# evalf/nutils

Measured on AMD Instinct MI355X. Metric: elements assembled/sec (global stiffness K), higher is better.
Workload: dtype f64; 1 GPU; 3D Poisson stiffness, 128^3 structured hex, p=1, 2x2x2 Gauss, iso geometry (BASELINE.json configs[1]); nelems_per_gpu=2097152, nnz_per_gpu=57066625, kernel=k_p1hex_skew<16,16,false,false>, parallelism=single GPU, launch=hipGraph replay (20 steps per graph), settle_steps=600

## Files before the change

### nutils_amd/csrc/nh_assemble_p1hex.hip

```cpp
#include "nh_common.h"
#include <algorithm>
#include <type_traits>
#include <cstdio>
#include <cstdlib>

namespace {

#ifdef NH_ABLATION
#define DEBUG(p) ((p).debug)
#else
#define DEBUG(p) 0
#endif

struct P1Args {
  int n0, n1, n2;
  int lay0, lay1;
  int pl0, pl1;
  const double *verts;
  double origin[3], scale[3];
  double n[2][2];
  double c[3][2];
  double wk[2][2][2];
  double wm[2][2][2];
  int hasm;
  const double *qmass;
  double *values;
  const double *qscale;
  const double *u;
  double *out;
  int accumulate;
  int nbj, nbk;
  long long *tdbg;
  int wbnd;
  int debug;
};

__device__ __forceinline__ int len_of(int X, int N) { return (X > 0) + 1 + (X < N - 1); }
__device__ __forceinline__ i64 cum_of(int X, int N) { return X == 0 ? 0 : 3 * (i64)X - 1; }

__device__ __forceinline__ double fast_rcp(double d) {
  double r = __builtin_amdgcn_rcp(d);
  r = fma(fma(-d, r, 1.), r, r);
  r = fma(fma(-d, r, 1.), r, r);
  return r;
}

__device__ __forceinline__ void lds_barrier() { asm volatile("s_waitcnt lgkmcnt(0)\n\ts_barrier" ::: "memory"); }

struct ElemTables {
  double R0[3][3], R1[3][3], R2[3][3];
  double W01[2][2][3], W02[2][2][3], W12[2][2][3];
  double Mm[3][3][3];
};

__device__ __forceinline__ double element_entry(const ElemTables &T, int a, int bb) {
  const int a0 = a >> 2, a1 = (a >> 1) & 1, a2 = a & 1;
  const int b0 = bb >> 2, b1 = (bb >> 1) & 1, b2 = bb & 1;
  const int p0 = a0 + b0, p1 = a1 + b1, p2 = a2 + b2;
  const double s00 = (a0 == b0) ? 1. : -1., s11 = (a1 == b1) ? 1. : -1., s22 = (a2 == b2) ? 1. : -1.;
  const double s01 = (a0 == b1) ? 1. : -1., s10 = (b0 == a1) ? 1. : -1.;
  const double s02 = (a0 == b2) ? 1. : -1., s20 = (b0 == a2) ? 1. : -1.;
  const double s12 = (a1 == b2) ? 1. : -1., s21 = (b1 == a2) ? 1. : -1.;
  return s00 * T.R0[p1][p2] + s11 * T.R1[p0][p2] + s22 * T.R2[p0][p1] + s01 * T.W01[b0][a1][p2] + s10 * T.W01[a0][b1][p2] +
         s02 * T.W02[b0][a2][p1] + s20 * T.W02[a0][b2][p1] + s12 * T.W12[b1][a2][p0] + s21 * T.W12[a1][b2][p0] + T.Mm[p0][p1][p2];
}

template <int TJ, int TK, int L, int VPT, int VW>
__device__ __forceinline__ void load_vertex_tile(const P1Args &p, bool valid, int J0, int K0, int L0, int tid, double (&V)[VPT][VW]) {
  constexpr int NT = L * TJ * TK, VJ = TJ + 1, VK = TK + 1, NV = (L + 1) * VJ * VK;
  const int N0 = p.n0 + 1, N1 = p.n1 + 1, N2 = p.n2 + 1;
#pragma unroll
  for (int k = 0; k < VPT; ++k) {
    const int v = tid + k * NT;
    const int c = v % VK, bb = (v / VK) % VJ, a = v / (VK * VJ);
    const int I = L0 + a, J = J0 - 1 + bb, K = K0 - 1 + c;
#pragma unroll
    for (int w = 0; w < VW; ++w) V[k][w] = 0.;
    if (valid && v < NV && I >= 0 && I < N0 && J >= 0 && J < N1 && K >= 0 && K < N2) {
      const i64 node = ((i64)I * N1 + J) * N2 + K;
      const double *src = p.verts + node * 3;
      V[k][0] = src[0];
      V[k][1] = src[1];
      V[k][2] = src[2];
      if constexpr (VW == 4) V[k][3] = p.u[node];
    }
  }
}

template <int TJ, int TK, int L, bool VEC, bool MASS, bool COEF>
__global__ __launch_bounds__(L * TJ * TK) void k_p1hex_march(P1Args p) {
#ifdef NH_ABLATION
  long long tacc[12] = {0, 0, 0, 0, 0, 0, 0, 0, 0, 0, 0, 0}, tprev = clock64();
#define NH_TICK(i) { const long long tnow = clock64(); tacc[i] += tnow - tprev; tprev = tnow; }
#else
#define NH_TICK(i)
#endif
  constexpr int NT = L * TJ * TK, NP = L + 2, OJ = TJ - 1, OK = TK - 1;
  constexpr int NS = VEC ? 1 : 15;
  constexpr int VW = VEC ? 4 : 3;
  constexpr int VJ = TJ + 1, VK = TK + 1, RP = VJ * VK, PS = (RP * NS + 1) & ~1, NV = (L + 1) * VJ * VK, VPT = (NV + NT - 1) / NT;
  extern __shared__ __attribute__((aligned(16))) double lds[];
  double *acc = lds;
  double *vbuf = lds + NP * PS;
  const int tid = threadIdx.x;
  const int N0 = p.n0 + 1, N1 = p.n1 + 1, N2 = p.n2 + 1;
  const int NPL = p.pl1 - p.pl0;
  const i64 U = (i64)p.nbj * p.nbk * NPL;
  const unsigned wg = gridDim.x % 8 == 0 ? (blockIdx.x % 8) * (gridDim.x / 8) + blockIdx.x / 8 : blockIdx.x;
  i64 u = U * wg / gridDim.x;
  const i64 u1 = U * (wg + 1) / gridDim.x;
  if (u >= u1) return;
  auto slot_of = [](int P) { return (int)((unsigned)(P + 2 * NP) % NP) * PS; };
  int col = (int)(u / NPL), A = p.pl0 + (int)(u % NPL), B = (int)min((i64)p.pl1, A + (u1 - u)), L0 = A - 1;
  double V[VPT][VW];
  load_vertex_tile<TJ, TK, L, VPT, VW>(p, true, (col / p.nbk) * OJ, (col % p.nbk) * OK, L0, tid, V);
  for (int t = tid; t < NP * PS / 2; t += NT) reinterpret_cast<double2 *>(acc)[t] = make_double2(0., 0.);
  auto stage_vertex_tile = [&]() {
#pragma unroll
    for (int k = 0; k < VPT; ++k) {
// ... 148 lines not shown
          const int nl = half ? 7 : 8;
          if (l < 202) {
#pragma unroll
            for (int pl = 0; pl < 2; ++pl) {
              char *lp = base + pl * (8 * (3 * T1 * T2)) + 16 * l;
#pragma unroll
              for (int i = 0; i < 8; ++i)
                if (i < nl) {
                  const double2 v = make_double2(a0[pl][i], a1[pl][i]);
                  __builtin_memcpy(lp + i * (2 * stride8), &v, 16);
                }
            }
          } else if (l == 202) {
#pragma unroll
            for (int pl = 0; pl < 2; ++pl) {
              char *lp = base + pl * (8 * (3 * T1 * T2)) + 16 * l;
#pragma unroll
              for (int i = 0; i < 8; ++i)
                if (i < nl) *reinterpret_cast<double *>(lp + i * (2 * stride8)) = a0[pl][i];
            }
          }
        } else if (L == 2 && !lowJ && !highJ && Pe - Pb == 2 && Pb > 0 && Pe < N0) {
          const int flag = 1 | 2 | loK << 2 | 8 | 16 | hiK << 5;
          const unsigned voff8 = 8u * (unsigned)(9 * cumK + ((dI + 1) * 3 + (dJ + 1)) * lenK + (dK + loK));
          const i64 stride8 = 8 * (i64)(9 * (int)T2);
          if (kact && (flag & need) == need) {
            const bool below = !upper && dI < 0;
            const double *src0 = acc + (below ? slot_of(Pb - 1) : slot_of(Pb)) + srow, *src1 = acc + (below ? slot_of(Pb) : slot_of(Pb + 1)) + srow;
            double v0[OJ], v1[OJ];
#pragma unroll
            for (int oj = 0; oj < OJ; ++oj) v0[oj] = src0[oj * (VK * NS)];
#pragma unroll
            for (int oj = 0; oj < OJ; ++oj) v1[oj] = src1[oj * (VK * NS)];
            char *lp0 = reinterpret_cast<char *>(p.values + ((3 * (i64)Pb - 1) * T1 * T2 + 3 * (cumJ0 * T2)));
            char *lp1 = lp0 + 8 * (3 * T1 * T2);
#pragma unroll
            for (int oj = 0; oj < OJ; ++oj) {
              *reinterpret_cast<double *>(lp0 + voff8) = v0[oj];
              lp0 += stride8;
            }
#pragma unroll
            for (int oj = 0; oj < OJ; ++oj) {
              *reinterpret_cast<double *>(lp1 + voff8) = v1[oj];
              lp1 += stride8;
            }
          }
        } else if (!lowJ && !highJ) planes(std::integral_constant<int, 0>{});
        else if (!(lowJ && highJ)) planes(std::integral_constant<int, 1>{});
        else planes(std::integral_constant<int, 2>{});
      }
    }
    NH_TICK(4)
    if (last) break;
    lds_barrier();
    NH_TICK(5)
    if (fresh) {
      for (int t = tid; t < NP * PS / 2; t += NT) reinterpret_cast<double2 *>(acc)[t] = make_double2(0., 0.);
    } else {
#pragma unroll
      for (int P = L0 - 1; P < L0 + L - 1; ++P) {
        double2 *z = reinterpret_cast<double2 *>(acc + slot_of(P));
        for (int t = tid; t < PS / 2; t += NT) z[t] = make_double2(0., 0.);
      }
    }
    col = ncol, A = nA, B = nB, L0 = nL0;
    NH_TICK(6)
  }
#ifdef NH_ABLATION
  if (p.tdbg && (tid & 63) == 0)
    for (int i = 0; i < 8; ++i) atomicAdd((unsigned long long *)p.tdbg + i, (unsigned long long)tacc[i]);
#endif
}
#undef NH_TICK

__device__ __forceinline__ void half_arrive(unsigned *cnt) {
  asm volatile("s_waitcnt lgkmcnt(0)" ::: "memory");
  if ((threadIdx.x & 63) == 0) atomicAdd(cnt, 1u);
}
__device__ __forceinline__ void half_wait(unsigned *cnt, unsigned target) {
  while (__hip_atomic_load(cnt, __ATOMIC_RELAXED, __HIP_MEMORY_SCOPE_WORKGROUP) < target) __builtin_amdgcn_s_sleep(1);
  asm volatile("" ::: "memory");
}

template <int TJ, int TK, bool MASS, bool COEF>
__global__ __launch_bounds__(2 * TJ * TK) void k_p1hex_skew(P1Args p) {
  constexpr bool VEC = false;
#ifdef NH_ABLATION
  long long tacc[10] = {0, 0, 0, 0, 0, 0, 0, 0, 0, 0}, tprev = clock64();
  const long long tstart = tprev;
  int nslow = 0, nfast = 0;
#ifdef NH_NOTICKS
#define NH_TICK(i)
#else
#define NH_TICK(i) { const long long tnow = clock64(); tacc[i] += tnow - tprev; tprev = tnow; }
#endif
#else
#define NH_TICK(i)
#endif
  constexpr int G = TJ * TK, NT = 2 * G, NP = 4, OJ = TJ - 1, OK = TK - 1, NS = 15, VW = 3;
  constexpr int VJ = TJ + 1, VK = TK + 1, RP = VJ * VK, PS = (RP * NS + 1) & ~1, VPG = (RP + G - 1) / G;
  const bool getenv_stage_late = p.wbnd < 0;
  extern __shared__ __attribute__((aligned(16))) double lds[];
  double *acc = lds;
  double *vbuf = lds + NP * PS;
  unsigned *hcnt = reinterpret_cast<unsigned *>(vbuf + 3 * RP * VW);
  const int tid = threadIdx.x, lt = tid & (G - 1), grp = __builtin_amdgcn_readfirstlane(tid / G);
  const int N0 = p.n0 + 1, N1 = p.n1 + 1, N2 = p.n2 + 1;
  const int NPL = p.pl1 - p.pl0;
  const unsigned wg = gridDim.x % 8 == 0 ? (blockIdx.x % 8) * (gridDim.x / 8) + blockIdx.x / 8 : blockIdx.x;
  const i64 CP = NPL + 2, WI = 16, WB = p.nbj > 1 ? (p.wbnd < 0 ? -p.wbnd : p.wbnd) : 16;
  const i64 rowB = p.nbk * CP * WB, rowI = p.nbk * CP * WI, nmid = max(p.nbj - 2, 0);
  const i64 ctot = (p.nbj > 1 ? 2 : 1) * rowB + nmid * rowI;
  auto unit_at = [&](i64 c) {
    i64 jt, rem, w;
    if (c < rowB) jt = 0, rem = c, w = WB;
    else if (c < rowB + nmid * rowI) jt = 1 + (c - rowB) / rowI, rem = (c - rowB) % rowI, w = WI;
    else jt = p.nbj > 1 ? p.nbj - 1 : 1, rem = c - rowB - nmid * rowI, w = WB;
    const i64 kt = rem / (CP * w), pos = (rem - kt * CP * w) / w;
    return (jt * p.nbk + kt) * NPL + min(max(pos - 1, (i64)0), (i64)NPL);
  };
  i64 u = unit_at(ctot * wg / gridDim.x);
  const i64 u1 = unit_at(ctot * (wg + 1) / gridDim.x);
  if (u >= u1) return;
  auto slot_of = [](int P) { return (int)((unsigned)(P + 2 * NP) % NP) * PS; };
  auto vslot_of = [](int P) { return (int)((unsigned)(P + 3) % 3) * (RP * VW); };
  auto load_vertex = [&](int I, int r, int J0, int K0, double (&x)[3]) {
    const int bb = r / VK, c = r % VK, J = J0 - 1 + bb, K = K0 - 1 + c;
    x[0] = x[1] = x[2] = 0.;
    if (r < RP && I >= 0 && I < N0 && J >= 0 && J < N1 && K >= 0 && K < N2) {
      const double *src = p.verts + (((i64)I * N1 + J) * N2 + K) * 3;
      x[0] = src[0], x[1] = src[1], x[2] = src[2];
    }
  };
  if (tid == 0) *hcnt = 0;
  unsigned htarget = 0;
  const i64 T1 = 3 * (i64)N1 - 2, T2 = 3 * (i64)N2 - 2;
  while (u < u1) {
    const int col = (int)(u / NPL), A = p.pl0 + (int)(u % NPL), B = (int)min((i64)p.pl1, A + (u1 - u));
    const int J0 = (col / p.nbk) * OJ, K0 = (col % p.nbk) * OK;
    {
      constexpr int NVL = (2 * RP + NT - 1) / NT;
      double x[NVL][3];
      bool valid[NVL];
#pragma unroll
      for (int k = 0; k < NVL; ++k) {
        const int v = min(tid + k * NT, 2 * RP - 1), pl = v / RP, r = v % RP, I = A - 1 + pl;
        const int J = J0 - 1 + r / VK, K = K0 - 1 + r % VK;
        valid[k] = I >= 0 && I < N0 && J >= 0 && J < N1 && K >= 0 && K < N2;
        const double *src = p.verts + (((i64)min(max(I, 0), N0 - 1) * N1 + min(max(J, 0), N1 - 1)) * N2 + min(max(K, 0), N2 - 1)) * 3;
        x[k][0] = src[0], x[k][1] = src[1], x[k][2] = src[2];
      }
      for (int t = tid; t < NP * PS / 2; t += NT) reinterpret_cast<double2 *>(acc)[t] = make_double2(0., 0.);
#pragma unroll
      for (int k = 0; k < NVL; ++k) {
        const int v = tid + k * NT, pl = v / RP, r = v % RP;
        if (v < 2 * RP) {
          double *dst = vbuf + vslot_of(A - 1 + pl) + r * VW;
          dst[0] = valid[k] ? x[k][0] : 0., dst[1] = valid[k] ? x[k][1] : 0., dst[2] = valid[k] ? x[k][2] : 0.;
        }
      }
    }
    lds_barrier();

    for (int s = A - 1; s <= B; ++s) {
      htarget += G / 64;
      NH_TICK(0)
      const bool mathrole = ((s - (A - 1)) & 1) == grp;
      if (mathrole) {
        const int ej = lt / TK, ek = lt % TK;
        const int gi = s, gj = J0 - 1 + ej, gk = K0 - 1 + ek;
        if (s < B && gi >= p.lay0 && gi < p.lay1 && gj >= 0 && gj < p.n1 && gk >= 0 && gk < p.n2 && !(DEBUG(p) & 4)) {
#define NH_P1HEX_VERT(a, bb, c) (vbuf + vslot_of(gi + (a)) + ((ej + (bb)) * VK + (ek + (c))) * VW)
#include "nh_p1hex_element.inc"
#undef NH_P1HEX_VERT
        }
        NH_TICK(3)
      } else {
        const bool needv = s + 1 < B && !(DEBUG(p) & 8);
        double Vn[VPG][3];
#pragma unroll
        for (int k = 0; k < VPG; ++k) load_vertex(needv ? s + 2 : -1, lt + k * G, J0, K0, Vn[k]);
        const int P = s - 1;
        bool arrived = false, staged = false;
        auto stage_vertices = [&]() {
#pragma unroll
          for (int k = 0; k < VPG; ++k) {
            const int r = lt + k * G;
            if (r < RP) {
              double *dst = vbuf + vslot_of(s + 2) + r * VW;
              dst[0] = Vn[k][0], dst[1] = Vn[k][1], dst[2] = Vn[k][2];
            }
          }
        };
        if (P >= A && !(DEBUG(p) & 2)) {
          const bool lowJ = J0 == 0, highJ = J0 + OJ >= N1;
          const int cumJ0 = J0 == 0 ? 0 : 3 * J0 - 1;
#ifdef NH_ABLATION
          if (!lowJ && !highJ && P > 0 && P < N0 - 1 && K0 > 0 && K0 + OK < N2) ++nfast; else ++nslow;
#endif
          if (!lowJ && !highJ && P > 0 && P < N0 - 1 && K0 > 0 && K0 + OK < N2) {
            const int e = 2 * lt;
            auto source = [&](int ee, bool &below) {
              const int ok_ = ee / 27, sl_ = ee - ok_ * 27;
              const int dJ_ = (sl_ / 3) % 3 - 1, dK_ = sl_ % 3 - 1;
              below = sl_ < 9;
              return (VK + ok_ + 1) * NS + (sl_ >= 13 ? sl_ - 13 : (dJ_ * VK + dK_) * NS + 13 - sl_);
            };
            bool belowA, belowB;
            const int offA = source(e < 405 ? e : 404, belowA), offB = source(e + 1 < 405 ? e + 1 : 404, belowB);
            const double *sA = acc + (belowA ? slot_of(P - 1) : slot_of(P)) + offA;
            const double *sB = acc + (belowB ? slot_of(P - 1) : slot_of(P)) + offB;
            double a0[OJ], a1[OJ];
#pragma unroll
            for (int i = 0; i < OJ; ++i) {
              a0[i] = sA[i * (VK * NS)];
              a1[i] = sB[i * (VK * NS)];
            }
            const int li = lt - 202;
            const bool lone = li >= 0 && li < OJ;
            bool belowL;
            const int offL = source(404, belowL);
            const double aL = acc[(belowL ? slot_of(P - 1) : slot_of(P)) + offL + (lone ? li : 0) * (VK * NS)];
            half_arrive(hcnt);
            arrived = true;
            NH_TICK(8)
            if (needv && !getenv_stage_late) {
              __builtin_amdgcn_s_waitcnt(0x0f70);
              stage_vertices();
              staged = true;
            }
            const i64 stride8 = 8 * (i64)(9 * (int)T2);
            char *l0 = reinterpret_cast<char *>(p.values + ((3 * (i64)P - 1) * T1 * T2 + 3 * (cumJ0 * T2) + 9 * (3 * (i64)K0 - 1)));
            char *lp = l0 + 16 * lt;
            if (lt < 202) {
#pragma unroll
              for (int i = 0; i < OJ; ++i) {
                if ((DEBUG(p) & 16) && (i & 1)) continue;
                const double2 v = make_double2(a0[i], a1[i]);
                __builtin_memcpy(lp + i * stride8, &v, 16);
              }
            }
            if (lone) *reinterpret_cast<double *>(l0 + li * stride8 + 8 * 404) = aL;
          } else {
            constexpr int RPP = G / 32, KP = (OK + RPP - 1) / RPP;
            const int sl = lt & 31, rsub = lt >> 5;
            const int dI = sl / 9 - 1, dJ = (sl / 3) % 3 - 1, dK = sl % 3 - 1;
            const bool upper = sl >= 13;
            const int need = (dI < 0 ? 1 : dI > 0 ? 8 : 0) | (dJ < 0 ? 2 : dJ > 0 ? 16 : 0) | (dK < 0 ? 4 : dK > 0 ? 32 : 0);
            const int loI = P > 0, hiI = P < N0 - 1, lenI = loI + 1 + hiI;
            double v[KP][OJ];
#pragma unroll
            for (int kp = 0; kp < KP; ++kp) {
              const int ok = kp * RPP + rsub;
              const int srow = (VK + ok + 1) * NS + (upper ? sl - 13 : (dJ * VK + dK) * NS + 13 - sl);
              const double *src = acc + ((!upper && dI < 0) ? slot_of(P - 1) : slot_of(P)) + (ok < OK ? srow : 0);
#pragma unroll
              for (int oj = 0; oj < OJ; ++oj) v[kp][oj] = src[oj * (VK * NS)];
            }
            half_arrive(hcnt);
            arrived = true;
#pragma unroll
            for (int kp = 0; kp < KP; ++kp) {
              const int ok = kp * RPP + rsub, Kk = K0 + ok;
              const bool kact = sl < 27 && ok < OK && Kk < N2;
              const int loK = Kk > 0, hiK = Kk < N2 - 1, lenK = loK + 1 + hiK, cumK = Kk == 0 ? 0 : 3 * Kk - 1;
              double *line = p.values + ((P == 0 ? 0 : 3 * (i64)P - 1) * T1 * T2 + lenI * (cumJ0 * T2));
              if (!lowJ && !highJ) {
                const int flag = loI | 2 | loK << 2 | hiI << 3 | 16 | hiK << 5;
                const unsigned voff8 = 8u * (unsigned)(lenI * 3 * cumK + ((dI + loI) * 3 + (dJ + 1)) * lenK + (dK + loK));
                const i64 stride8 = 8 * (i64)(lenI * 3 * (int)T2);
                if (kact && (flag & need) == need) {
                  char *lp = reinterpret_cast<char *>(line);
#pragma unroll
                  for (int oj = 0; oj < OJ; ++oj) {
                    if (!((DEBUG(p) & 16) && (oj & 1))) *reinterpret_cast<double *>(lp + voff8) = v[kp][oj];
                    lp += stride8;
                  }
                }
              } else {
#pragma unroll
                for (int oj = 0; oj < OJ; ++oj) {
                  const int J = J0 + oj;
                  const int loJ = J > 0, hiJ = J < N1 - 1, lenJ = loJ + 1 + hiJ;
                  const int flag = loI | loJ << 1 | loK << 2 | hiI << 3 | hiJ << 4 | hiK << 5;
                  const unsigned voff = (unsigned)(lenI * lenJ * cumK + ((dI + loI) * lenJ + (dJ + loJ)) * lenK + (dK + loK));
                  if (kact && J < N1 && (flag & need) == need && !((DEBUG(p) & 16) && (oj & 1))) line[voff] = v[kp][oj];
                  line += lenI * lenJ * (int)T2;
                }
              }
            }
          }
        }
        NH_TICK(6)
        if (!arrived) half_arrive(hcnt);
        half_wait(hcnt, htarget);
        NH_TICK(7)
        {
          double2 *z = reinterpret_cast<double2 *>(acc + slot_of(s - 2));
          for (int t = lt; t < PS / 2; t += G) z[t] = make_double2(0., 0.);
        }
        NH_TICK(9)
        if (needv && !staged) stage_vertices();
      }
      if (mathrole) { NH_TICK(1) } else { NH_TICK(4) }
      lds_barrier();
      if (mathrole) { NH_TICK(2) } else { NH_TICK(5) }
    }
    u += B - A;
  }
#ifdef NH_ABLATION
  if (p.tdbg && tid == 0) {
    p.tdbg[16 + 4 * blockIdx.x] = clock64() - tstart;
    p.tdbg[16 + 4 * blockIdx.x + 1] = nfast;
    p.tdbg[16 + 4 * blockIdx.x + 2] = nslow;
  }
  if (p.tdbg && (tid & 63) == 0)
    for (int i = 0; i < 10; ++i) atomicAdd((unsigned long long *)p.tdbg + i, (unsigned long long)tacc[i]);
#endif
}
#undef NH_TICK

__global__ void k_p1hex_unit_matrix(P1Args p, double *Ke) {
  double X[2][2][2][3];
  for (int a = 0; a < 2; ++a)
    for (int b = 0; b < 2; ++b)
      for (int c = 0; c < 2; ++c) {
        X[a][b][c][0] = p.origin[0] + p.scale[0] * a;
        X[a][b][c][1] = p.origin[1] + p.scale[1] * b;
        X[a][b][c][2] = p.origin[2] + p.scale[2] * c;
      }
  ElemTables T;
  {
    double (&R0)[3][3] = T.R0, (&R1)[3][3] = T.R1, (&R2)[3][3] = T.R2;
    double (&W01)[2][2][3] = T.W01, (&W02)[2][2][3] = T.W02, (&W12)[2][2][3] = T.W12;
    double (&Mm)[3][3][3] = T.Mm;
    for (int i = 0; i < 27; ++i) (&Mm[0][0][0])[i] = 0.;
    const bool hasm = p.hasm;
#define NH_P1HEX_QS(q) 1.
#define NH_P1HEX_QM(q) 1.
#include "nh_p1hex_math.inc"
#undef NH_P1HEX_QS
#undef NH_P1HEX_QM
  }
#pragma unroll
  for (int a = 0; a < 8; ++a)
#pragma unroll
    for (int b = 0; b < 8; ++b) Ke[a * 8 + b] = element_entry(T, a < b ? a : b, a < b ? b : a);
}

__global__ __launch_bounds__(256) void k_p1hex_uniform(P1Args p, const double *KeG) {
  __shared__ double Ke[64], tabI[2 * 27], tabF[18], tabL[18];
  if (threadIdx.x < 64) Ke[threadIdx.x] = KeG[threadIdx.x];
  __syncthreads();
  const int N0 = p.n0 + 1, N1 = p.n1 + 1, N2 = p.n2 + 1;
  const int I = p.pl0 + blockIdx.x / N1, J = blockIdx.x % N1;
  const i64 T1 = 3 * (i64)N1 - 2, T2 = 3 * (i64)N2 - 2;
  const int lenI = len_of(I, N0), lenJ = len_of(J, N1), R3 = lenI * lenJ * 3, R2 = lenI * lenJ * 2;
  double *const line = p.values + (cum_of(I, N0) * T1 * T2 + lenI * (cum_of(J, N1) * T2));
  const int sl = threadIdx.x;
  if (sl < 27) {
    const int dI = sl / 9 - 1, dJ = (sl / 3) % 3 - 1, dK = sl % 3 - 1;
    const int cI = I + dI, cJ = J + dJ;
    if (cI >= 0 && cI < N0 && cJ >= 0 && cJ < N1) {
      double w[2][2];
#pragma unroll
      for (int a2 = 0; a2 < 2; ++a2)
#pragma unroll
        for (int b2 = 0; b2 < 2; ++b2) {
          double v = 0.;
#pragma unroll
          for (int oi = -1; oi <= 0; ++oi) {
            const int i = I + oi, a0 = -oi, b0 = a0 + dI;
            if (b0 < 0 || b0 > 1 || i < p.lay0 || i >= p.lay1) continue;
#pragma unroll
            for (int oj = -1; oj <= 0; ++oj) {
              const int j = J + oj, a1 = -oj, b1 = a1 + dJ;
              if (b1 < 0 || b1 > 1 || j < 0 || j >= p.n1) continue;
              v += Ke[((a0 * 2 + a1) * 2 + a2) * 8 + (b0 * 2 + b1) * 2 + b2];
            }
          }
          w[a2][b2] = v;
        }
      const int prefix = (dI + (I > 0)) * lenJ + (dJ + (J > 0));
      double v = 0.;
      if (dK <= 0) v += w[1][1 + dK];
      if (dK >= 0) v += w[0][dK];
      tabI[prefix * 3 + (dK + 1)] = v;
      tabI[R3 + prefix * 3 + (dK + 1)] = v;
      if (dK >= 0) tabF[prefix * 2 + dK] = w[0][dK];
      if (dK <= 0) tabL[prefix * 2 + (dK + 1)] = w[1][1 + dK];
    }
  }
  __syncthreads();
  const int ninner = (N2 - 2) * R3;
  double *const inner = line + R2;
  const int head = (int)((reinterpret_cast<size_t>(inner) >> 3) & 1);
  const int npairs = (ninner - head) / 2;
  int r = (head + 2 * (int)threadIdx.x) % R3;
  const int step = 512 % R3;
  double2 *const dst = reinterpret_cast<double2 *>(inner + head);
  for (int e = threadIdx.x; e < npairs; e += 256) {
    dst[e] = make_double2(tabI[r], tabI[r + 1]);
    r += step;
    r -= r >= R3 ? R3 : 0;
  }
  if (threadIdx.x == 0 && head) inner[0] = tabI[0];
  if (threadIdx.x == 1 && ((ninner - head) & 1)) inner[ninner - 1] = tabI[(ninner - 1) % R3];
  if (threadIdx.x < R2) {
    line[threadIdx.x] = tabF[threadIdx.x];
    line[R2 + ninner + threadIdx.x] = tabL[threadIdx.x];
  }
}

__global__ void k_p1hex_pattern(int n0, int n1, int n2, i64 row0, i64 row1, i64 *rowptr, i64 *colidx) {
  const int N0 = n0 + 1, N1 = n1 + 1, N2 = n2 + 1;
  const i64 t = (i64)blockIdx.x * blockDim.x + threadIdx.x;
  const i64 row = row0 + t / 27;
  const int slot = (int)(t % 27);
  if (row > row1 || (row == row1 && slot != 0)) return;
  const i64 T1 = 3 * (i64)N1 - 2, T2 = 3 * (i64)N2 - 2;
  auto rp = [&](i64 r) -> i64 {
    if (r >= (i64)N0 * N1 * N2) return (3 * (i64)N0 - 2) * T1 * T2;
    const int Kk = (int)(r % N2), J = (int)((r / N2) % N1), I = (int)(r / ((i64)N2 * N1));
    return cum_of(I, N0) * T1 * T2 + len_of(I, N0) * (cum_of(J, N1) * T2 + (i64)len_of(J, N1) * cum_of(Kk, N2));
  };
  const i64 base = rp(row0);
  if (slot == 0) rowptr[row - row0] = rp(row) - base;
  if (row >= row1) return;
  const int Kk = (int)(row % N2), J = (int)((row / N2) % N1), I = (int)(row / ((i64)N2 * N1));
  const int dI = slot / 9 - 1, dJ = (slot / 3) % 3 - 1, dK = slot % 3 - 1;
  const int cI = I + dI, cJ = J + dJ, cK = Kk + dK;
  if (cI < 0 || cI >= N0 || cJ < 0 || cJ >= N1 || cK < 0 || cK >= N2) return;
  const int lenJ = len_of(J, N1), lenK = len_of(Kk, N2);
  const int pos = ((dI + (I > 0)) * lenJ + (dJ + (J > 0))) * lenK + (dK + (Kk > 0));
  colidx[rp(row) - base + pos] = ((i64)cI * N1 + cJ) * N2 + cK;
}

}

template <bool VEC, bool MASS, bool COEF>
static int launch_march_inst(const nh_p1hex_args *a, P1Args &p, void *stream) {
#ifdef NH_ABLATION
  p.debug = getenv("NH_P1HEX_DEBUG") ? atoi(getenv("NH_P1HEX_DEBUG")) : 0;
#endif
  p.wbnd = 20;
#ifdef NH_ABLATION
  static const int wbnd_env = getenv("NH_P1HEX_WBND") ? std::min(64, std::max(8, atoi(getenv("NH_P1HEX_WBND")))) : 20;
  p.wbnd = getenv("NH_P1HEX_STAGE_LATE") ? -wbnd_env : wbnd_env;
#endif
  constexpr int TJ = 16, TK = 16, L = 2, NTM = L * TJ * TK, NS = VEC ? 1 : 15, VW = VEC ? 4 : 3;
  int dev = 0;
  NH_CHECK_HIP(hipGetDevice(&dev));
  NH_REQUIRE(dev >= 0 && dev < 16, "nh_p1hex: device index %d not supported", dev);
  static int cus_of[16] = {0};
  if (!cus_of[dev]) {
    int n = 256;
    NH_CHECK_HIP(hipDeviceGetAttribute(&n, hipDeviceAttributeMultiprocessorCount, dev));
    cus_of[dev] = n;
  }
  const int cus = cus_of[dev];
  p.nbj = (p.n1 + 1 + TJ - 2) / (TJ - 1);
  p.nbk = (p.n2 + 1 + TK - 2) / (TK - 1);
  const size_t ldsm = sizeof(double) * ((L + 2) * (((TJ + 1) * (TK + 1) * NS + 1) & ~1) + (L + 1) * (TJ + 1) * (TK + 1) * VW + 2);
  const i64 units = (i64)p.nbj * p.nbk * (p.pl1 - p.pl0);
  NH_REQUIRE(a->max_workgroups >= 0, "nh_p1hex: negative max_workgroups");
  unsigned grid = (unsigned)std::min<i64>(units, a->max_workgroups ? std::min(cus, a->max_workgroups) : cus);
#ifdef NH_ABLATION
  if (getenv("NH_P1HEX_MAXWG")) grid = std::min<unsigned>(grid, (unsigned)atoi(getenv("NH_P1HEX_MAXWG")));
#endif
  auto kern = k_p1hex_march<TJ, TK, L, VEC, MASS, COEF>;
  if constexpr (!VEC && L == 2) {
    const char *env = getenv("NH_P1HEX_KERNEL");
    if (!(env && !strcmp(env, "march"))) kern = k_p1hex_skew<TJ, TK, MASS, COEF>;
  }
  static const void *attr_set[16][2] = {{nullptr, nullptr}};
  if (attr_set[dev][0] != (const void *)kern && attr_set[dev][1] != (const void *)kern) {
    NH_CHECK_HIP(hipFuncSetAttribute((const void *)kern, hipFuncAttributeMaxDynamicSharedMemorySize, (int)ldsm));
    attr_set[dev][attr_set[dev][0] ? 1 : 0] = (const void *)kern;
  }
#ifdef NH_ABLATION
  static long long *tdbg = nullptr;
  if (!tdbg) NH_CHECK_HIP(hipMalloc((void **)&tdbg, (16 + 4 * 1024) * sizeof(long long)));
  NH_CHECK_HIP(hipMemsetAsync(tdbg, 0, (16 + 4 * 1024) * sizeof(long long), nh_stream(stream)));
  p.tdbg = getenv("NH_P1HEX_TIMERS") ? tdbg : nullptr;
#endif
  hipLaunchKernelGGL(kern, dim3(grid), dim3(NTM), ldsm, nh_stream(stream), p);
  NH_LAUNCH_CHECK();
#ifdef NH_ABLATION
  if (p.tdbg) {
    static long long h[16 + 4 * 1024];
    NH_CHECK_HIP(hipMemcpy(h, tdbg, sizeof h, hipMemcpyDeviceToHost));
    if (getenv("NH_P1HEX_WGTIMES"))
      for (unsigned g = 0; g < grid; ++g) fprintf(stderr, "wg %u cycles %lld fast %lld slow %lld\n", g, h[16 + 4 * g], h[16 + 4 * g + 1], h[16 + 4 * g + 2]);
    const double nw = (double)grid * (NTM / 64);
    if (kern != (void (*)(P1Args))k_p1hex_march<TJ, TK, L, VEC, MASS, COEF>)
      fprintf(stderr, "p1hex_skew cycles per wave: prologue %.0f | math %.0f | - %.0f | math wait %.0f | lds reads %.0f | store issue %.0f | half wait %.0f | zero %.0f | stage %.0f | mem wait %.0f\n", h[0] / nw, h[3] / nw, h[1] / nw,
              h[2] / nw, h[8] / nw, h[6] / nw, h[7] / nw, h[9] / nw, h[4] / nw, h[5] / nw);
    else
    fprintf(stderr, "p1hex_march cycles per wave: stage+next %.0f | B1 %.0f | load+math %.0f | B2 %.0f | stage+flush %.0f | B3 %.0f | zero %.0f\n", h[0] / nw, h[1] / nw,
            h[2] / nw, h[3] / nw, h[4] / nw, h[5] / nw, h[6] / nw);
  }
#endif
  return NH_OK;
}

template <bool VEC>
static int launch_march(const nh_p1hex_args *a, P1Args &p, void *stream) {
  const bool coef = p.qscale || p.qmass;
  if (p.hasm) return coef ? launch_march_inst<VEC, true, true>(a, p, stream) : launch_march_inst<VEC, true, false>(a, p, stream);
  return coef ? launch_march_inst<VEC, false, true>(a, p, stream) : launch_march_inst<VEC, false, false>(a, p, stream);
}

extern "C" {

int nh_p1hex_pattern(const int *shape, int64_t row_begin, int64_t row_end, int64_t *rowptr_dev, int64_t *colidx_dev, void *stream) {
  NH_REQUIRE(shape && rowptr_dev && colidx_dev, "nh_p1hex_pattern: NULL argument");
  NH_REQUIRE(shape[0] >= 1 && shape[1] >= 1 && shape[2] >= 1, "nh_p1hex_pattern: empty mesh");
  const i64 nrows_total = (i64)(shape[0] + 1) * (shape[1] + 1) * (shape[2] + 1);
  NH_REQUIRE(0 <= row_begin && row_begin <= row_end && row_end <= nrows_total, "nh_p1hex_pattern: row range out of bounds");
  const i64 n = (row_end - row_begin + 1) * 27;
  hipLaunchKernelGGL(k_p1hex_pattern, dim3((unsigned)((n + 255) / 256)), dim3(256), 0, nh_stream(stream), shape[0], shape[1], shape[2],
                     (i64)row_begin, (i64)row_end, (i64 *)rowptr_dev, (i64 *)colidx_dev);
  NH_LAUNCH_CHECK();
  return NH_OK;
}

static int fill_p1args(const nh_p1hex_args *a, P1Args &p) {
  NH_REQUIRE(a, "nh_p1hex: NULL argument");
  NH_REQUIRE(a->shape[0] >= 1 && a->shape[1] >= 1 && a->shape[2] >= 1, "nh_p1hex: empty mesh");
  NH_REQUIRE(0 <= a->layer_begin && a->layer_begin <= a->layer_end && a->layer_end <= a->shape[0], "nh_p1hex: layer range");
  NH_REQUIRE(0 <= a->plane_begin && a->plane_begin <= a->plane_end && a->plane_end <= a->shape[0] + 1, "nh_p1hex: plane range");
  NH_REQUIRE(fabs(a->gauss_x[0] + a->gauss_x[1] - 1.) <= 1e-14, "nh_p1hex: gauss_x must be a symmetric 2-point rule (gauss_x[0] + gauss_x[1] = 1)");
  p.n0 = a->shape[0];
  p.n1 = a->shape[1];
  p.n2 = a->shape[2];
  p.lay0 = a->layer_begin;
  p.lay1 = a->layer_end;
  p.pl0 = a->plane_begin;
  p.pl1 = a->plane_end;
  p.verts = a->verts_dev;
  for (int d = 0; d < 3; ++d) {
    p.origin[d] = a->origin[d];
    p.scale[d] = a->scale[d];
  }
  for (int q = 0; q < 2; ++q) {
    p.n[0][q] = 1. - a->gauss_x[q];
    p.n[1][q] = a->gauss_x[q];
    p.c[0][q] = p.n[0][q] * p.n[0][q];
    p.c[1][q] = p.n[0][q] * p.n[1][q];
    p.c[2][q] = p.n[1][q] * p.n[1][q];
  }
  for (int qa = 0; qa < 2; ++qa)
    for (int qb = 0; qb < 2; ++qb)
      for (int qc = 0; qc < 2; ++qc) {
        p.wk[qa][qb][qc] = a->kappa * a->gauss_w[qa] * a->gauss_w[qb] * a->gauss_w[qc];
        p.wm[qa][qb][qc] = a->mass * a->gauss_w[qa] * a->gauss_w[qb] * a->gauss_w[qc];
      }
  p.hasm = a->mass != 0. || a->qmass_dev != nullptr;
  p.qmass = a->qmass_dev;
  p.values = a->values_dev;
  p.qscale = a->qscale_dev;
  p.u = nullptr;
  p.out = nullptr;
  p.accumulate = 0;
  p.nbj = p.nbk = 0;
  p.debug = 0;
  p.wbnd = 16;
  p.tdbg = nullptr;
  return NH_OK;
}

int nh_p1hex_unit_matrix(const nh_p1hex_args *a, double *ke_dev, void *stream) {
  NH_REQUIRE(ke_dev, "nh_p1hex_unit_matrix: NULL output");
  P1Args p;
  int rc = fill_p1args(a, p);
  if (rc) return rc;
  hipLaunchKernelGGL(k_p1hex_unit_matrix, dim3(1), dim3(1), 0, nh_stream(stream), p, ke_dev);
  NH_LAUNCH_CHECK();
// ... 40 lines not shown
```

### nutils_amd/csrc/nh_p1hex_math.inc

```
{
  const double (&n)[2][2] = p.n;
  const double (&c)[3][2] = p.c;
  double J0[2][2][3], J1[2][2][3], J2[2][2][3];
#pragma unroll
  for (int d = 0; d < 3; ++d) {
    double e0[2][2], e1[2][2], e2[2][2];
#pragma unroll
    for (int x = 0; x < 2; ++x)
#pragma unroll
      for (int y = 0; y < 2; ++y) {
        e0[x][y] = X[1][x][y][d] - X[0][x][y][d];
        e1[x][y] = X[x][1][y][d] - X[x][0][y][d];
        e2[x][y] = X[x][y][1][d] - X[x][y][0][d];
      }
    double t0[2][2], t1[2][2], t2[2][2];
#pragma unroll
    for (int y = 0; y < 2; ++y) {
      const double d0 = e0[1][y] - e0[0][y], d1 = e1[1][y] - e1[0][y], d2 = e2[1][y] - e2[0][y];
#pragma unroll
      for (int q1 = 0; q1 < 2; ++q1) {
        t0[q1][y] = fma(n[1][q1], d0, e0[0][y]);
        t1[q1][y] = fma(n[1][q1], d1, e1[0][y]);
        t2[q1][y] = fma(n[1][q1], d2, e2[0][y]);
      }
    }
#pragma unroll
    for (int q1 = 0; q1 < 2; ++q1) {
      const double d0 = t0[q1][1] - t0[q1][0], d1 = t1[q1][1] - t1[q1][0], d2 = t2[q1][1] - t2[q1][0];
#pragma unroll
      for (int q2 = 0; q2 < 2; ++q2) {
        J0[q1][q2][d] = fma(n[1][q2], d0, t0[q1][0]);
        J1[q1][q2][d] = fma(n[1][q2], d1, t1[q1][0]);
        J2[q1][q2][d] = fma(n[1][q2], d2, t2[q1][0]);
      }
    }
  }
  double D0[2][2], D1[2][2], D2[2][2], M01[2][2][2], M02[2][2][2], M12[2][2][2], Dm[2][2][2];
#pragma unroll
  for (int qa = 0; qa < 2; ++qa)
#pragma unroll
    for (int qb = 0; qb < 2; ++qb)
#pragma unroll
      for (int qc = 0; qc < 2; ++qc) {
        const double *c0 = J0[qb][qc], *c1 = J1[qa][qc], *c2 = J2[qa][qb];
        double A[3][3];
        A[0][0] = c1[1] * c2[2] - c1[2] * c2[1];
        A[0][1] = c1[2] * c2[0] - c1[0] * c2[2];
        A[0][2] = c1[0] * c2[1] - c1[1] * c2[0];
        A[1][0] = c2[1] * c0[2] - c2[2] * c0[1];
        A[1][1] = c2[2] * c0[0] - c2[0] * c0[2];
        A[1][2] = c2[0] * c0[1] - c2[1] * c0[0];
        A[2][0] = c0[1] * c1[2] - c0[2] * c1[1];
        A[2][1] = c0[2] * c1[0] - c0[0] * c1[2];
        A[2][2] = c0[0] * c1[1] - c0[1] * c1[0];
        const double det = c0[0] * A[0][0] + c0[1] * A[0][1] + c0[2] * A[0][2];
        const double sc = p.wk[qa][qb][qc] * NH_P1HEX_QS(qa * 4 + qb * 2 + qc) * fast_rcp(fabs(det));
        const double m00 = sc * (A[0][0] * A[0][0] + A[0][1] * A[0][1] + A[0][2] * A[0][2]);
        const double m11 = sc * (A[1][0] * A[1][0] + A[1][1] * A[1][1] + A[1][2] * A[1][2]);
        const double m22 = sc * (A[2][0] * A[2][0] + A[2][1] * A[2][1] + A[2][2] * A[2][2]);
        M01[qa][qb][qc] = sc * (A[0][0] * A[1][0] + A[0][1] * A[1][1] + A[0][2] * A[1][2]);
        M02[qa][qb][qc] = sc * (A[0][0] * A[2][0] + A[0][1] * A[2][1] + A[0][2] * A[2][2]);
        M12[qa][qb][qc] = sc * (A[1][0] * A[2][0] + A[1][1] * A[2][1] + A[1][2] * A[2][2]);
        D0[qb][qc] = qa ? D0[qb][qc] + m00 : m00;
        D1[qa][qc] = qb ? D1[qa][qc] + m11 : m11;
        D2[qa][qb] = qc ? D2[qa][qb] + m22 : m22;
        if (hasm) Dm[qa][qb][qc] = p.wm[qa][qb][qc] * NH_P1HEX_QM(qa * 4 + qb * 2 + qc) * fabs(det);
      }
  const double al = n[0][0], nal = -al, c00 = c[0][0], c01 = c[0][1], c10 = c[1][0], cs = c00 + c01;
#define NH_P1HEX_LERP(o0, o1, u0, u1) \
  {                                   \
    const double d_ = (u0) - (u1);    \
    o0 = fma(al, d_, u1);             \
    o1 = fma(nal, d_, u0);            \
  }
#define NH_P1HEX_PAIR(o0, o1, o2, x, y) \
  {                                     \
    const double s_ = (x) + (y);        \
    o0 = fma(c00, x, c01 * (y));        \
    o1 = c10 * s_;                      \
    o2 = fma(cs, s_, -(o0));            \
  }
  {
    double U[2][3];
#pragma unroll
    for (int x = 0; x < 2; ++x) NH_P1HEX_PAIR(U[x][0], U[x][1], U[x][2], D0[x][0], D0[x][1])
#pragma unroll
    for (int p2 = 0; p2 < 3; ++p2) NH_P1HEX_PAIR(R0[0][p2], R0[1][p2], R0[2][p2], U[0][p2], U[1][p2])
#pragma unroll
    for (int x = 0; x < 2; ++x) NH_P1HEX_PAIR(U[x][0], U[x][1], U[x][2], D1[x][0], D1[x][1])
#pragma unroll
    for (int p2 = 0; p2 < 3; ++p2) NH_P1HEX_PAIR(R1[0][p2], R1[1][p2], R1[2][p2], U[0][p2], U[1][p2])
#pragma unroll
    for (int x = 0; x < 2; ++x) NH_P1HEX_PAIR(U[x][0], U[x][1], U[x][2], D2[x][0], D2[x][1])
#pragma unroll
    for (int p1 = 0; p1 < 3; ++p1) NH_P1HEX_PAIR(R2[0][p1], R2[1][p1], R2[2][p1], U[0][p1], U[1][p1])
  }
  {
    double V[2][2][2], V2[2][2][2];
#pragma unroll
    for (int be = 0; be < 2; ++be)
#pragma unroll
      for (int ga = 0; ga < 2; ++ga) NH_P1HEX_LERP(V[0][be][ga], V[1][be][ga], M01[0][be][ga], M01[1][be][ga])
#pragma unroll
    for (int b0 = 0; b0 < 2; ++b0)
#pragma unroll
      for (int ga = 0; ga < 2; ++ga) NH_P1HEX_LERP(V2[b0][0][ga], V2[b0][1][ga], V[b0][0][ga], V[b0][1][ga])
#pragma unroll
    for (int b0 = 0; b0 < 2; ++b0)
#pragma unroll
      for (int a1 = 0; a1 < 2; ++a1) NH_P1HEX_PAIR(W01[b0][a1][0], W01[b0][a1][1], W01[b0][a1][2], V2[b0][a1][0], V2[b0][a1][1])
#pragma unroll
    for (int be = 0; be < 2; ++be)
#pragma unroll
      for (int ga = 0; ga < 2; ++ga) NH_P1HEX_LERP(V[0][be][ga], V[1][be][ga], M02[0][be][ga], M02[1][be][ga])
#pragma unroll
    for (int b0 = 0; b0 < 2; ++b0)
#pragma unroll
      for (int be = 0; be < 2; ++be) NH_P1HEX_LERP(V2[b0][0][be], V2[b0][1][be], V[b0][be][0], V[b0][be][1])
#pragma unroll
    for (int b0 = 0; b0 < 2; ++b0)
#pragma unroll
      for (int a2 = 0; a2 < 2; ++a2) NH_P1HEX_PAIR(W02[b0][a2][0], W02[b0][a2][1], W02[b0][a2][2], V2[b0][a2][0], V2[b0][a2][1])
#pragma unroll
    for (int al_ = 0; al_ < 2; ++al_)
#pragma unroll
      for (int ga = 0; ga < 2; ++ga) NH_P1HEX_LERP(V[0][al_][ga], V[1][al_][ga], M12[al_][0][ga], M12[al_][1][ga])
#pragma unroll
    for (int b1 = 0; b1 < 2; ++b1)
#pragma unroll
      for (int al_ = 0; al_ < 2; ++al_) NH_P1HEX_LERP(V2[b1][0][al_], V2[b1][1][al_], V[b1][al_][0], V[b1][al_][1])
#pragma unroll
    for (int b1 = 0; b1 < 2; ++b1)
#pragma unroll
      for (int a2 = 0; a2 < 2; ++a2) NH_P1HEX_PAIR(W12[b1][a2][0], W12[b1][a2][1], W12[b1][a2][2], V2[b1][a2][0], V2[b1][a2][1])
  }
#undef NH_P1HEX_LERP
#undef NH_P1HEX_PAIR
  if (hasm) {
    double t1[2][2][3], t2[2][3][3];
#pragma unroll
    for (int qa = 0; qa < 2; ++qa)
#pragma unroll
      for (int qb = 0; qb < 2; ++qb)
#pragma unroll
        for (int p2 = 0; p2 < 3; ++p2) t1[qa][qb][p2] = c[p2][0] * Dm[qa][qb][0] + c[p2][1] * Dm[qa][qb][1];
#pragma unroll
    for (int qa = 0; qa < 2; ++qa)
#pragma unroll
      for (int p1 = 0; p1 < 3; ++p1)
#pragma unroll
        for (int p2 = 0; p2 < 3; ++p2) t2[qa][p1][p2] = c[p1][0] * t1[qa][0][p2] + c[p1][1] * t1[qa][1][p2];
#pragma unroll
    for (int p0 = 0; p0 < 3; ++p0)
#pragma unroll
      for (int p1 = 0; p1 < 3; ++p1)
#pragma unroll
        for (int p2 = 0; p2 < 3; ++p2) Mm[p0][p1][p2] = c[p0][0] * t2[0][p1][p2] + c[p0][1] * t2[1][p1][p2];
  }
}
```

Before: 12.17 billion elements/s.

## Precompute work split on host, hoist per-tile invariants, specialize uniform quadrature weights

Moves the per-workgroup work-split computation, which used i64 divisions, out of the skew kernel into a host-built cut table passed as a kernel argument. It also hoists per-column-tile invariants (lane validity bits, vertex offsets, the output base offset) out of the plane loop and rotates the LDS vertex slots by pointer swap instead of modulo. A template flag specializes the kernel when all quadrature weights are equal so the weight table lookup becomes a scalar. The changes are meant to cut integer ALU and scalar overhead in the prologue and inner loop. In exchange the kernel argument grows by about 3 KB and the grid is capped by the table size.

```diff
diff --git a/nutils_amd/csrc/nh_assemble_p1hex.hip b/nutils_amd/csrc/nh_assemble_p1hex.hip
--- a/nutils_amd/csrc/nh_assemble_p1hex.hip
+++ b/nutils_amd/csrc/nh_assemble_p1hex.hip
@@ -1,4 +1,5 @@
 #include "nh_common.h"
+#include "nh_p1hex_split.inc"
 #include <algorithm>
 #include <type_traits>
 #include <cstdio>
@@ -35,6 +36,10 @@
   int debug;
 };
 
+struct P1Cuts {
+  int32_t u[NH_P1HEX_MAXGRID][2];
+};
+
 __device__ __forceinline__ int len_of(int X, int N) { return (X > 0) + 1 + (X < N - 1); }
 __device__ __forceinline__ i64 cum_of(int X, int N) { return X == 0 ? 0 : 3 * (i64)X - 1; }
 
@@ -349,8 +354,8 @@
   asm volatile("" ::: "memory");
 }
 
-template <int TJ, int TK, bool MASS, bool COEF>
-__global__ __launch_bounds__(2 * TJ * TK) void k_p1hex_skew(P1Args p) {
+template <int TJ, int TK, bool MASS, bool COEF, bool WK1>
+__global__ __launch_bounds__(2 * TJ * TK) void k_p1hex_skew(P1Args p, P1Cuts cuts) {
   constexpr bool VEC = false;
 #ifdef NH_ABLATION
   long long tacc[10] = {0, 0, 0, 0, 0, 0, 0, 0, 0, 0}, tprev = clock64();
@@ -374,37 +379,39 @@
   const int tid = threadIdx.x, lt = tid & (G - 1), grp = __builtin_amdgcn_readfirstlane(tid / G);
   const int N0 = p.n0 + 1, N1 = p.n1 + 1, N2 = p.n2 + 1;
   const int NPL = p.pl1 - p.pl0;
-  const unsigned wg = gridDim.x % 8 == 0 ? (blockIdx.x % 8) * (gridDim.x / 8) + blockIdx.x / 8 : blockIdx.x;
-  const i64 CP = NPL + 2, WI = 16, WB = p.nbj > 1 ? (p.wbnd < 0 ? -p.wbnd : p.wbnd) : 16;
-  const i64 rowB = p.nbk * CP * WB, rowI = p.nbk * CP * WI, nmid = max(p.nbj - 2, 0);
-  const i64 ctot = (p.nbj > 1 ? 2 : 1) * rowB + nmid * rowI;
-  auto unit_at = [&](i64 c) {
-    i64 jt, rem, w;
-    if (c < rowB) jt = 0, rem = c, w = WB;
-    else if (c < rowB + nmid * rowI) jt = 1 + (c - rowB) / rowI, rem = (c - rowB) % rowI, w = WI;
-    else jt = p.nbj > 1 ? p.nbj - 1 : 1, rem = c - rowB - nmid * rowI, w = WB;
-    const i64 kt = rem / (CP * w), pos = (rem - kt * CP * w) / w;
-    return (jt * p.nbk + kt) * NPL + min(max(pos - 1, (i64)0), (i64)NPL);
-  };
-  i64 u = unit_at(ctot * wg / gridDim.x);
-  const i64 u1 = unit_at(ctot * (wg + 1) / gridDim.x);
-  if (u >= u1) return;
-  auto slot_of = [](int P) { return (int)((unsigned)(P + 2 * NP) % NP) * PS; };
-  auto vslot_of = [](int P) { return (int)((unsigned)(P + 3) % 3) * (RP * VW); };
-  auto load_vertex = [&](int I, int r, int J0, int K0, double (&x)[3]) {
-    const int bb = r / VK, c = r % VK, J = J0 - 1 + bb, K = K0 - 1 + c;
-    x[0] = x[1] = x[2] = 0.;
-    if (r < RP && I >= 0 && I < N0 && J >= 0 && J < N1 && K >= 0 && K < N2) {
-      const double *src = p.verts + (((i64)I * N1 + J) * N2 + K) * 3;
-      x[0] = src[0], x[1] = src[1], x[2] = src[2];
-    }
-  };
+  unsigned u = (unsigned)cuts.u[blockIdx.x][0];
+  const unsigned u1 = (unsigned)cuts.u[blockIdx.x][1];
+  asm volatile("" ::"s"(p.n0), "s"(p.n[1][0]), "s"(p.c[0][0]), "s"(p.values), "s"(p.nbk));
+  static_assert((NP & (NP - 1)) == 0, "slot_of masks the plane number");
+  auto slot_of = [](int P) { return (P & (NP - 1)) * PS; };
+  constexpr int LB_ELEM = 1, LB_VERT = 2 , LB_PAIR = 1 << (1 + VPG), LB_LONE = 2 << (1 + VPG), LB_STAGE = 4 << (1 + VPG) ;
+  const int ej = lt / TK, ek = lt % TK;
   if (tid == 0) *hcnt = 0;
   unsigned htarget = 0;
   const i64 T1 = 3 * (i64)N1 - 2, T2 = 3 * (i64)N2 - 2;
+  const i64 pstride = 3 * T1 * T2;
   while (u < u1) {
-    const int col = (int)(u / NPL), A = p.pl0 + (int)(u % NPL), B = (int)min((i64)p.pl1, A + (u1 - u));
-    const int J0 = (col / p.nbk) * OJ, K0 = (col % p.nbk) * OK;
+    const unsigned col = u / (unsigned)NPL, pin = u - col * (unsigned)NPL, jt = col / (unsigned)p.nbk;
+    const int A = p.pl0 + (int)pin, B = A + (int)min(u1 - u, (unsigned)NPL - pin);
+    const int J0 = (int)jt * OJ, K0 = (int)(col - jt * (unsigned)p.nbk) * OK;
+    const bool lowJ = J0 == 0, highJ = J0 + OJ >= N1, inner = !lowJ && !highJ && K0 > 0 && K0 + OK < N2;
+    const int cumJ0 = J0 == 0 ? 0 : 3 * J0 - 1;
+    i64 foff = (3 * (i64)(A - 2) - 1) * T1 * T2 + 3 * (cumJ0 * T2) + 9 * (3 * (i64)K0 - 1);
+    int vs0 = 0, vs1 = RP * VW, vs2 = 2 * RP * VW;
+    int lanebits = (lt < 202 ? LB_PAIR : 0) | (lt >= 202 && lt < 202 + OJ ? LB_LONE : 0);
+    {
+      const int gj = J0 - 1 + ej, gk = K0 - 1 + ek;
+      if (gj >= 0 && gj < p.n1 && gk >= 0 && gk < p.n2) lanebits |= LB_ELEM;
+    }
+    i64 voff[VPG];
+#pragma unroll
+    for (int k = 0; k < VPG; ++k) {
+      const int r = lt + k * G, J = J0 - 1 + r / VK, K = K0 - 1 + r % VK;
+      const bool ok = r < RP && J >= 0 && J < N1 && K >= 0 && K < N2;
+      if (ok) lanebits |= LB_VERT << k;
+      if (r < RP) lanebits |= LB_STAGE << k;
+      voff[k] = ok ? ((i64)J * N2 + K) * 3 : 0;
+    }
     {
       constexpr int NVL = (2 * RP + NT - 1) / NT;
       double x[NVL][3];
@@ -422,50 +429,59 @@
       for (int k = 0; k < NVL; ++k) {
         const int v = tid + k * NT, pl = v / RP, r = v % RP;
         if (v < 2 * RP) {
-          double *dst = vbuf + vslot_of(A - 1 + pl) + r * VW;
+          double *dst = vbuf + (pl ? vs1 : vs0) + r * VW;
           dst[0] = valid[k] ? x[k][0] : 0., dst[1] = valid[k] ? x[k][1] : 0., dst[2] = valid[k] ? x[k][2] : 0.;
         }
       }
     }
     lds_barrier();
 
-    for (int s = A - 1; s <= B; ++s) {
+    for (int s = A - 1, sn; s <= B; s = sn) {
+      sn = s + 1;
       htarget += G / 64;
       NH_TICK(0)
       const bool mathrole = ((s - (A - 1)) & 1) == grp;
+      int lb = lanebits;
+      asm volatile("" : "+v"(lb));
       if (mathrole) {
-        const int ej = lt / TK, ek = lt % TK;
         const int gi = s, gj = J0 - 1 + ej, gk = K0 - 1 + ek;
-        if (s < B && gi >= p.lay0 && gi < p.lay1 && gj >= 0 && gj < p.n1 && gk >= 0 && gk < p.n2 && !(DEBUG(p) & 4)) {
-#define NH_P1HEX_VERT(a, bb, c) (vbuf + vslot_of(gi + (a)) + ((ej + (bb)) * VK + (ek + (c))) * VW)
+        if (s < B && gi >= p.lay0 && gi < p.lay1 && !(DEBUG(p) & 4) && (lb & LB_ELEM)) {
+#define NH_P1HEX_VERT(a, bb, c) (vbuf + ((a) ? vs1 : vs0) + ((ej + (bb)) * VK + (ek + (c))) * VW)
+#define NH_P1HEX_WK(qa, qb, qc) (WK1 ? p.wk[0][0][0] : p.wk[qa][qb][qc])
 #include "nh_p1hex_element.inc"
+#undef NH_P1HEX_WK
 #undef NH_P1HEX_VERT
         }
         NH_TICK(3)
       } else {
-        const bool needv = s + 1 < B && !(DEBUG(p) & 8);
+        const bool needv = sn < B && !(DEBUG(p) & 8);
         double Vn[VPG][3];
-#pragma unroll
-        for (int k = 0; k < VPG; ++k) load_vertex(needv ? s + 2 : -1, lt + k * G, J0, K0, Vn[k]);
+        const double *vplane = p.verts + (i64)(s + 2) * N1 * N2 * 3;
+#pragma unroll
+        for (int k = 0; k < VPG; ++k) {
+          Vn[k][0] = Vn[k][1] = Vn[k][2] = 0.;
+          if (needv && s + 2 < N0 && (lb & (LB_VERT << k))) {
+            const double *src = vplane + voff[k];
+            Vn[k][0] = src[0], Vn[k][1] = src[1], Vn[k][2] = src[2];
+          }
+        }
         const int P = s - 1;
         bool arrived = false, staged = false;
         auto stage_vertices = [&]() {
 #pragma unroll
           for (int k = 0; k < VPG; ++k) {
             const int r = lt + k * G;
-            if (r < RP) {
-              double *dst = vbuf + vslot_of(s + 2) + r * VW;
+            if (lb & (LB_STAGE << k)) {
+              double *dst = vbuf + vs2 + r * VW;
               dst[0] = Vn[k][0], dst[1] = Vn[k][1], dst[2] = Vn[k][2];
             }
           }
         };
         if (P >= A && !(DEBUG(p) & 2)) {
-          const bool lowJ = J0 == 0, highJ = J0 + OJ >= N1;
-          const int cumJ0 = J0 == 0 ? 0 : 3 * J0 - 1;
-#ifdef NH_ABLATION
-          if (!lowJ && !highJ && P > 0 && P < N0 - 1 && K0 > 0 && K0 + OK < N2) ++nfast; else ++nslow;
-#endif
-          if (!lowJ && !highJ && P > 0 && P < N0 - 1 && K0 > 0 && K0 + OK < N2) {
+#ifdef NH_ABLATION
+          if (inner && P > 0 && P < N0 - 1) ++nfast; else ++nslow;
+#endif
+          if (inner && P > 0 && P < N0 - 1) {
             const int e = 2 * lt;
             auto source = [&](int ee, bool &below) {
               const int ok_ = ee / 27, sl_ = ee - ok_ * 27;
@@ -484,7 +500,7 @@
               a1[i] = sB[i * (VK * NS)];
             }
             const int li = lt - 202;
-            const bool lone = li >= 0 && li < OJ;
+            const bool lone = lb & LB_LONE;
             bool belowL;
             const int offL = source(404, belowL);
             const double aL = acc[(belowL ? slot_of(P - 1) : slot_of(P)) + offL + (lone ? li : 0) * (VK * NS)];
@@ -497,14 +513,16 @@
               staged = true;
             }
             const i64 stride8 = 8 * (i64)(9 * (int)T2);
-            char *l0 = reinterpret_cast<char *>(p.values + ((3 * (i64)P - 1) * T1 * T2 + 3 * (cumJ0 * T2) + 9 * (3 * (i64)K0 - 1)));
-            char *lp = l0 + 16 * lt;
-            if (lt < 202) {
+            char *l0 = reinterpret_cast<char *>(p.values + foff);
+            if (lb & LB_PAIR) {
+              i64 lo = 8 * foff;
 #pragma unroll
               for (int i = 0; i < OJ; ++i) {
-                if ((DEBUG(p) & 16) && (i & 1)) continue;
                 const double2 v = make_double2(a0[i], a1[i]);
-                __builtin_memcpy(lp + i * stride8, &v, 16);
+                if (!((DEBUG(p) & 16) && (i & 1)))
+                  __builtin_memcpy(reinterpret_cast<char *>(p.values) + lo + (unsigned)(16 * lt), &v, 16);
+                lo += stride8;
+                asm volatile("" : "+s"(lo));
               }
             }
             if (lone) *reinterpret_cast<double *>(l0 + li * stride8 + 8 * 404) = aL;
@@ -572,8 +590,11 @@
       if (mathrole) { NH_TICK(1) } else { NH_TICK(4) }
       lds_barrier();
       if (mathrole) { NH_TICK(2) } else { NH_TICK(5) }
-    }
-    u += B - A;
+      foff += pstride;
+      const int vs = vs0;
+      vs0 = vs1, vs1 = vs2, vs2 = vs;
+    }
+    u += (unsigned)(B - A);
   }
 #ifdef NH_ABLATION
   if (p.tdbg && tid == 0) {
@@ -735,15 +756,25 @@
 #ifdef NH_ABLATION
   if (getenv("NH_P1HEX_MAXWG")) grid = std::min<unsigned>(grid, (unsigned)atoi(getenv("NH_P1HEX_MAXWG")));
 #endif
-  auto kern = k_p1hex_march<TJ, TK, L, VEC, MASS, COEF>;
+  const void *kern = (const void *)k_p1hex_march<TJ, TK, L, VEC, MASS, COEF>;
+  bool skew = false, wk1 = true;
+  for (int q = 1; q < 8; ++q) wk1 = wk1 && (&p.wk[0][0][0])[q] == p.wk[0][0][0];
+  P1Cuts cuts;
   if constexpr (!VEC && L == 2) {
     const char *env = getenv("NH_P1HEX_KERNEL");
-    if (!(env && !strcmp(env, "march"))) kern = k_p1hex_skew<TJ, TK, MASS, COEF>;
-  }
-  static const void *attr_set[16][2] = {{nullptr, nullptr}};
-  if (attr_set[dev][0] != (const void *)kern && attr_set[dev][1] != (const void *)kern) {
-    NH_CHECK_HIP(hipFuncSetAttribute((const void *)kern, hipFuncAttributeMaxDynamicSharedMemorySize, (int)ldsm));
-    attr_set[dev][attr_set[dev][0] ? 1 : 0] = (const void *)kern;
+    if (!(env && !strcmp(env, "march"))) {
+      kern = wk1 ? (const void *)k_p1hex_skew<TJ, TK, MASS, COEF, true> : (const void *)k_p1hex_skew<TJ, TK, MASS, COEF, false>;
+      skew = true;
+      NH_REQUIRE(grid <= (unsigned)NH_P1HEX_MAXGRID, "nh_p1hex: %u workgroups exceed the work split table (%d)", grid, NH_P1HEX_MAXGRID);
+      NH_REQUIRE(units <= INT32_MAX, "nh_p1hex: %lld (column tile, plane) units do not fit 32 bits", (long long)units);
+      const bool fits = nh_p1hex_split_pairs(p.nbj, p.nbk, p.pl1 - p.pl0, p.wbnd, grid, cuts.u);
+      NH_REQUIRE(fits, "nh_p1hex: work split failed");
+    }
+  }
+  static const void *attr_set[16][3] = {{nullptr, nullptr, nullptr}};
+  if (attr_set[dev][0] != kern && attr_set[dev][1] != kern && attr_set[dev][2] != kern) {
+    NH_CHECK_HIP(hipFuncSetAttribute(kern, hipFuncAttributeMaxDynamicSharedMemorySize, (int)ldsm));
+    attr_set[dev][!attr_set[dev][0] ? 0 : !attr_set[dev][1] ? 1 : 2] = kern;
   }
 #ifdef NH_ABLATION
   static long long *tdbg = nullptr;
@@ -751,7 +782,11 @@
   NH_CHECK_HIP(hipMemsetAsync(tdbg, 0, (16 + 4 * 1024) * sizeof(long long), nh_stream(stream)));
   p.tdbg = getenv("NH_P1HEX_TIMERS") ? tdbg : nullptr;
 #endif
-  hipLaunchKernelGGL(kern, dim3(grid), dim3(NTM), ldsm, nh_stream(stream), p);
+  if constexpr (!VEC && L == 2) {
+    if (skew && wk1) hipLaunchKernelGGL((k_p1hex_skew<TJ, TK, MASS, COEF, true>), dim3(grid), dim3(NTM), ldsm, nh_stream(stream), p, cuts);
+    if (skew && !wk1) hipLaunchKernelGGL((k_p1hex_skew<TJ, TK, MASS, COEF, false>), dim3(grid), dim3(NTM), ldsm, nh_stream(stream), p, cuts);
+  }
+  if (!skew) hipLaunchKernelGGL((k_p1hex_march<TJ, TK, L, VEC, MASS, COEF>), dim3(grid), dim3(NTM), ldsm, nh_stream(stream), p);
   NH_LAUNCH_CHECK();
 #ifdef NH_ABLATION
   if (p.tdbg) {
@@ -760,7 +795,7 @@
     if (getenv("NH_P1HEX_WGTIMES"))
       for (unsigned g = 0; g < grid; ++g) fprintf(stderr, "wg %u cycles %lld fast %lld slow %lld\n", g, h[16 + 4 * g], h[16 + 4 * g + 1], h[16 + 4 * g + 2]);
     const double nw = (double)grid * (NTM / 64);
-    if (kern != (void (*)(P1Args))k_p1hex_march<TJ, TK, L, VEC, MASS, COEF>)
+    if (skew)
       fprintf(stderr, "p1hex_skew cycles per wave: prologue %.0f | math %.0f | - %.0f | math wait %.0f | lds reads %.0f | store issue %.0f | half wait %.0f | zero %.0f | stage %.0f | mem wait %.0f\n", h[0] / nw, h[3] / nw, h[1] / nw,
               h[2] / nw, h[8] / nw, h[6] / nw, h[7] / nw, h[9] / nw, h[4] / nw, h[5] / nw);
     else
diff --git a/nutils_amd/csrc/nh_p1hex_math.inc b/nutils_amd/csrc/nh_p1hex_math.inc
--- a/nutils_amd/csrc/nh_p1hex_math.inc
+++ b/nutils_amd/csrc/nh_p1hex_math.inc
@@ -1,3 +1,7 @@
+#ifndef NH_P1HEX_WK
+#define NH_P1HEX_WK(qa, qb, qc) p.wk[qa][qb][qc]
+#define NH_P1HEX_WK_IS_TABLE
+#endif
 {
   const double (&n)[2][2] = p.n;
   const double (&c)[3][2] = p.c;
@@ -54,7 +58,7 @@
         A[2][1] = c0[2] * c1[0] - c0[0] * c1[2];
         A[2][2] = c0[0] * c1[1] - c0[1] * c1[0];
         const double det = c0[0] * A[0][0] + c0[1] * A[0][1] + c0[2] * A[0][2];
-        const double sc = p.wk[qa][qb][qc] * NH_P1HEX_QS(qa * 4 + qb * 2 + qc) * fast_rcp(fabs(det));
+        const double sc = NH_P1HEX_WK(qa, qb, qc) * NH_P1HEX_QS(qa * 4 + qb * 2 + qc) * fast_rcp(fabs(det));
         const double m00 = sc * (A[0][0] * A[0][0] + A[0][1] * A[0][1] + A[0][2] * A[0][2]);
         const double m11 = sc * (A[1][0] * A[1][0] + A[1][1] * A[1][1] + A[1][2] * A[1][2]);
         const double m22 = sc * (A[2][0] * A[2][0] + A[2][1] * A[2][1] + A[2][2] * A[2][2]);
@@ -158,3 +162,7 @@
         for (int p2 = 0; p2 < 3; ++p2) Mm[p0][p1][p2] = c[p0][0] * t2[0][p1][p2] + c[p0][1] * t2[1][p1][p2];
   }
 }
+#ifdef NH_P1HEX_WK_IS_TABLE
+#undef NH_P1HEX_WK
+#undef NH_P1HEX_WK_IS_TABLE
+#endif
diff --git a/nutils_amd/csrc/nh_p1hex_split.inc b/nutils_amd/csrc/nh_p1hex_split.inc
--- /dev/null
+++ b/nutils_amd/csrc/nh_p1hex_split.inc
@@ -0,0 +1,34 @@
+#include <cstdint>
+
+constexpr int NH_P1HEX_MAXGRID = 384;
+
+static inline unsigned nh_p1hex_wg_of_block(unsigned b, unsigned grid) { return grid % 8 == 0 ? (b % 8) * (grid / 8) + b / 8 : b; }
+
+static inline bool nh_p1hex_split(int nbj, int nbk, int npl, int wbnd, unsigned grid, int32_t *cut) {
+  typedef long long i64;
+  if (nbj < 1 || nbk < 1 || npl < 1 || grid < 1 || grid > (unsigned)NH_P1HEX_MAXGRID || (i64)nbj * nbk * npl > INT32_MAX) return false;
+  const i64 CP = (i64)npl + 2, WI = 16, WB = nbj > 1 ? (wbnd < 0 ? -(i64)wbnd : wbnd) : 16;
+  const i64 rowB = nbk * CP * WB, rowI = nbk * CP * WI, nmid = nbj > 2 ? nbj - 2 : 0;
+  const i64 ctot = (nbj > 1 ? 2 : 1) * rowB + nmid * rowI;
+  for (unsigned g = 0; g <= grid; ++g) {
+    const i64 c = ctot * g / grid;
+    i64 jt, rem, w;
+    if (c < rowB) jt = 0, rem = c, w = WB;
+    else if (c < rowB + nmid * rowI) jt = 1 + (c - rowB) / rowI, rem = (c - rowB) % rowI, w = WI;
+    else jt = nbj > 1 ? nbj - 1 : 1, rem = c - rowB - nmid * rowI, w = WB;
+    const i64 kt = rem / (CP * w), pos = (rem - kt * CP * w) / w;
+    const i64 pl = pos - 1 < 0 ? 0 : pos - 1 > npl ? npl : pos - 1;
+    cut[g] = (int32_t)((jt * nbk + kt) * npl + pl);
+  }
+  return true;
+}
+
+static inline bool nh_p1hex_split_pairs(int nbj, int nbk, int npl, int wbnd, unsigned grid, int32_t (*pair)[2]) {
+  int32_t cut[NH_P1HEX_MAXGRID + 1];
+  if (!nh_p1hex_split(nbj, nbk, npl, wbnd, grid, cut)) return false;
+  for (unsigned b = 0; b < grid; ++b) {
+    const unsigned wg = nh_p1hex_wg_of_block(b, grid);
+    pair[b][0] = cut[wg], pair[b][1] = cut[wg + 1];
+  }
+  return true;
+}
```

Measured after the change: 12.13 billion elements/s. No clear change (-0.3%).
